# KelestZ/Latent2im

Measured on AMD Instinct MI355X. Metric: edited images/sec, higher is better.
Workload: dtype f32; 1 GPU; StyleGAN2 FFHQ-shaped 1024^2 generator (random-init, noise weights ~ 0.05: per-layer noise drawn every pass), ResNet-50 regressor, 1 CelebA attr (train.py flow), full loss (reg+content+GAN), batch 8 per GPU, linear W+ walk, eager launches; resolution=1024, global_batch=8, per_gpu_batch=8, losses=reg+content+gan, parallelism=dp1, loss_branch_streams=3, hip_graph=False

## Files before the change

include/l2i.h:

```cpp
#ifndef L2I_H
#define L2I_H

#include <stdint.h>

#ifdef __cplusplus
extern "C" {
#endif

#define L2I_OK 0
#define L2I_E_ARG (-1)
#define L2I_E_LAUNCH (-2)
#define L2I_E_UNSUPPORTED (-3)

#define L2I_ACT_NONE 0
#define L2I_ACT_LRELU 1
#define L2I_ACT_RELU 2

typedef struct l2i_conv_params {
    const float* x;
    const float* w;
    float* y;
    int32_t B, Cin, H, W, Cout, CoutP;
    int32_t KH, KW, stride, pad_y, pad_x;
    int32_t OH, OW, OHf, OWf;
// ... 28 lines not shown
    const float* rgb_bias;
    float* rgb_out;
    float* pool_out;
    uint8_t* pool_idx;
    uint8_t* mask_out;
    int32_t mask_bits;
} l2i_conv_params;
#define L2I_SQ_SLOTS 1024

int l2i_conv2d_f32(const l2i_conv_params* p, void* stream);

#define L2I_FAMILY_IMPLICIT_GEMM 0
#define L2I_FAMILY_GEMM1X1 1
#define L2I_FAMILY_CIN3 2
#define L2I_FAMILY_DIRECT_SMALL 3
int l2i_conv2d_family(const l2i_conv_params* p);

int l2i_conv_transpose2d_f32(const l2i_conv_params* p, void* stream);
#define L2I_CONVT_HINT_DIRECT 9
#define L2I_CONVT_HINT_POLY 10
#define L2I_TFAMILY_DIRECT 0
#define L2I_TFAMILY_POLY 1
#define L2I_TFAMILY_SMALL 2
int l2i_conv_transpose2d_family(const l2i_conv_params* p);
typedef struct l2i_convt_poly_plan {
    int32_t eligible, masked;
    int32_t nwx, nwy;
    int32_t WTW, WTH, tiles_x, tiles_y, mblocks;
    int32_t total, grid;
    int32_t IH, IW, org, nslots, plane, wpitch;
    int32_t CK, stage_floats, lds_bytes;
// ... 236 lines not shown
```

latent2im_amd/_lib.py:

```python
import ctypes
import os

import torch

_HERE = os.path.dirname(os.path.abspath(__file__))
LIB_PATH = os.environ.get('L2I_LIB') or os.path.join(_HERE, 'libl2i_hip.so')

ACT_NONE, ACT_LRELU, ACT_RELU = 0, 1, 2
LINEAR_NONE, LINEAR_LRELU, LINEAR_WALK = 0, 1, 2

c_f = ctypes.c_float
c_i = ctypes.c_int32
c_p = ctypes.c_void_p
c_l = ctypes.c_int64
c_d = ctypes.c_double


class ConvParams(ctypes.Structure):
    _fields_ = [
        ('x', c_p), ('w', c_p), ('y', c_p),
        ('B', c_i), ('Cin', c_i), ('H', c_i), ('W', c_i), ('Cout', c_i), ('CoutP', c_i),
        ('KH', c_i), ('KW', c_i), ('stride', c_i), ('pad_y', c_i), ('pad_x', c_i),
        ('OH', c_i), ('OW', c_i), ('OHf', c_i), ('OWf', c_i),
        ('oy_step', c_i), ('ox_step', c_i), ('oy_off', c_i), ('ox_off', c_i),
# ... 22 lines not shown

class SegmvSeg(ctypes.Structure):
    _fields_ = [('rows', c_i), ('nparts', c_i), ('out_off_c', c_i), ('out_off_b', c_i), ('out_bstride', c_i), ('epi', c_i), ('bias_off', c_i),
                ('e_off_c', c_i), ('e_off_b', c_i), ('e_bstride', c_i), ('rgb_off_b', c_i), ('rgb_w_off', c_i), ('part', SegmvPart * 2)]


CONVT_HINT_DIRECT, CONVT_HINT_POLY = 9, 10
TFAMILY_DIRECT, TFAMILY_POLY, TFAMILY_SMALL = 0, 1, 2


class ConvtPolyPlan(ctypes.Structure):
    _fields_ = [(n, c_i) for n in ('eligible', 'masked', 'nwx', 'nwy', 'WTW', 'WTH', 'tiles_x', 'tiles_y', 'mblocks', 'total', 'grid',
                                   'IH', 'IW', 'org', 'nslots', 'plane', 'wpitch', 'CK', 'stage_floats', 'lds_bytes')]


H8_EPI_LEAN, H8_EPI_GENERAL, H8_EPI_F32_VEC, H8_EPI_F32_SCALAR = 0, 1, 2, 3


class ConvH8Plan(ctypes.Structure):
    _fields_ = [(n, c_i) for n in ('eligible', 'WM', 'WN', 'KS', 'K', 'S', 'TR', 'out32', 'relu_in', 'extra', 'rgb', 'epilogue', 'nchunks', 'tiles_x',
                                   'tiles_y', 'mblocks', 'total', 'grid', 'lds_bytes')]


def conv_h8_plan(p, transposed=False):
    plan = ConvH8Plan()
    check(load().l2i_conv_h8_plan_for(ctypes.byref(p), int(bool(transposed)), ctypes.byref(plan)), 'l2i_conv_h8_plan_for')
    return plan


ADAM_MAX_TENSORS = 16
# ... 14 lines not shown

def repack_taps(taps):
    t = RepackTaps()
    t.count = len(taps)
    for i, (ky, kx) in enumerate(taps[:REPACK_MAX_TAPS]):
        t.ky[i], t.kx[i] = ky, kx
    return t


_SIGNATURES = {
    'l2i_conv2d_f32': (c_i, [ctypes.POINTER(ConvParams), c_p]),
    'l2i_conv2d_family': (c_i, [ctypes.POINTER(ConvParams)]),
    'l2i_conv_transpose2d_f32': (c_i, [ctypes.POINTER(ConvParams), c_p]),
    'l2i_conv_transpose2d_family': (c_i, [ctypes.POINTER(ConvParams)]),
    'l2i_convt_poly_plan_for': (c_i, [ctypes.POINTER(ConvParams), ctypes.POINTER(ConvtPolyPlan)]),
    'l2i_conv2d_bf16x3_f32': (c_i, [ctypes.POINTER(ConvParams), c_p]),
    'l2i_conv_transpose2d_bf16x3_f32': (c_i, [ctypes.POINTER(ConvParams), c_p]),
    'l2i_conv2d_wino_f32': (c_i, [ctypes.POINTER(ConvParams), c_p]),
    'l2i_conv2d_wino4_f32': (c_i, [ctypes.POINTER(ConvParams), c_p]),
    'l2i_wino4s_epilogue_class': (c_i, [ctypes.POINTER(ConvParams)]),
    'l2i_conv1x1_pair_f32': (c_i, [ctypes.POINTER(ConvParams), ctypes.POINTER(ConvParams), c_p]),
    'l2i_conv2d_h8': (c_i, [ctypes.POINTER(ConvParams), c_p]),
    'l2i_conv_transpose2d_h8': (c_i, [ctypes.POINTER(ConvParams), c_p]),
    'l2i_conv_h8_plan_for': (c_i, [ctypes.POINTER(ConvParams), c_i, ctypes.POINTER(ConvH8Plan)]),
    'l2i_conv_img_h8': (c_i, [ctypes.POINTER(ConvParams), c_p]),
    'l2i_conv1x1_pair_h8': (c_i, [ctypes.POINTER(ConvParams), ctypes.POINTER(ConvParams), c_i, c_p]),
    'l2i_conv_chain3_h8': (c_i, [ctypes.POINTER(ConvParams), ctypes.POINTER(ConvParams), ctypes.POINTER(ConvParams), c_i, c_p]),
    'l2i_fused_bias_act_f32': (c_i, [c_p, c_p, c_p, c_p, c_l, c_l, c_l, c_i, c_i, c_f, c_f, c_p]),
    'l2i_fused_bias_act_f16': (c_i, [c_p, c_p, c_p, c_p, c_l, c_l, c_l, c_i, c_i, c_f, c_f, c_p]),
    'l2i_upfirdn2d_f16': (c_i, [c_p, c_p, c_p, c_l, c_i, c_i, c_i, c_i, c_i, c_i, c_i, c_i, c_i, c_i, c_i, c_i, c_p]),
# ... 54 lines not shown
    'l2i_pixelnorm_act_h8': (c_i, [c_p, c_p, c_p, c_i, c_i, c_i, c_i, c_f, c_f, c_i, c_p]),
    'l2i_pixelnorm_act_bwd_h8': (c_i, [c_p, c_p, c_p, c_p, c_i, c_i, c_i, c_i, c_f, c_f, c_i, c_p]),
    'l2i_linear_rows_f32': (c_i, [c_p, c_p, c_p, c_p, c_p, c_p, c_i, c_i, c_i, c_i, c_f, c_p]),
    'l2i_linear_rows_bwd_f32': (c_i, [c_p, c_p, c_p, c_p, c_p, c_p, c_p, c_p, c_p, c_p, c_i, c_i, c_i, c_i, c_f, c_i, c_p]),
    'l2i_range_stats': (c_i, [c_p, c_p, c_l, c_i, c_p]),
    'l2i_last_error': (ctypes.c_char_p, []),
    'l2i_abi_version': (c_i, []),
    'l2i_sizeof_conv_params': (c_i, []),
}

_F16_TWINS = frozenset(k for k in _SIGNATURES if k.endswith('_h8') or k in ('l2i_cast_f32_to_h8', 'l2i_cast_h8_to_f32'))
for _n in [k for k in _SIGNATURES if k in _F16_TWINS]:
    _SIGNATURES[_n + '_f16'] = _SIGNATURES[_n]

ABI_VERSION = 12
ADDITIVE = frozenset(('l2i_conv_transpose2d_family', 'l2i_convt_poly_plan_for', 'l2i_conv_h8_plan_for', 'l2i_bn_finalize_f32', 'l2i_bn_bwd_finalize_f32',
                      'l2i_repack_taps_f32', 'l2i_repack_wino_f32', 'l2i_batch_from_u8_f32'))

EXPORTS = tuple(_SIGNATURES)

_lib = None


BUILD_HASHES = os.path.join(_HERE, 'csrc', 'BUILD_HASHES.json')


def committed_build():
    import hashlib
    import json
    try:
        with open(BUILD_HASHES) as f:
# ... 87 lines not shown
```

latent2im_amd/conv.py:

```python

import numpy as np
import torch

from . import _lib
from ._lib import ACT_LRELU, ACT_NONE, ACT_RELU, ConvParams


import os as _os

PRECISION = _os.environ.get('L2I_PRECISION', 'f32')
H8_PRECISIONS = ('bf16', 'f16')


def h8_dtype():
    return torch.float16 if PRECISION == 'f16' else torch.bfloat16

USE_WINOGRAD = True
WINO4_MODES = ('all', 'tall', 'r4', 'off')
WINO4 = 'all'
WINO4_R4_MIN_W = 64
SPLIT_K = True
_WS = {}
USE_FUSED_TRANSPOSED = True
PROFILE = None
FAMILIES = ('implicit_gemm_f32', 'gemm1x1_f32', 'cin3_f32', 'direct_small_valu')
FAMILY_INFO = {
    'winograd_f32': ('conv_wino_kernel', 16.0 / 36.0, 157.3),
    'winograd4_f32': ('conv_wino4s_kernel', 36.0 / 144.0, 157.3),
    'implicit_gemm_f32': ('conv_mfma_kernel / conv3x3s2_dma_kernel', 1.0, 157.3),
    'gemm1x1_f32': ('gemm1x1_kernel', 1.0, 157.3),
    'transposed_f32': ('convt_mfma_kernel', 1.0, 157.3),
    'transposed_poly_f32': ('convt_poly_kernel', 25.0 / 36.0, 157.3),
    'cin3_f32': ('conv_cin3_kernel', 28.0 / 27.0, 157.3),
    'direct_small_valu': ('conv_direct_small_kernel', 1.0, 157.3),
    'implicit_gemm_bf16x3': ('conv_bf16x3_pipe_kernel', 3.0, 2500.0),
    'transposed_bf16x3': ('conv_bf16x3_pipe_kernel<TR>', 3.0, 2500.0),
    'conv_h8': ('conv_h8_kernel', 1.0, 2500.0),
    'transposed_h8': ('conv_h8_kernel<TR>', 1.0, 2500.0),
}


def pack_weight(w):
    w = torch.as_tensor(w, dtype=torch.float32)
    cout, cin, kh, kw = w.shape
# ... 55 lines not shown
_POLY_G = np.array([[0, 0, 1], [1, 0, 1], [1, 0, 0], [0, 1, 0], [0, 1, 0]], dtype=np.float64)


def pack_weight_convt_poly(w, dtype=torch.float32):
    w = torch.as_tensor(w, dtype=torch.float64)
    cout, cin, kh, kw = w.shape
    assert kh == 3 and kw == 3
    G = torch.as_tensor(_POLY_G, device=w.device)
    U = torch.einsum('ik,ockl,jl->ocij', G, w, G)
    coutp = (cout + 31) // 32 * 32
    p = torch.zeros(cin, 25, coutp, dtype=dtype, device=w.device)
    p[:, :, :cout] = U.permute(1, 2, 3, 0).reshape(cin, 25, cout).to(dtype)
    return p.contiguous()


def _bf16x3_planes(self):
    if self.w16 is None and self.w_src is not None:
        hi, lo = pack_weight_bf16x3(self.w_src)
        self.w16 = (hi.to(self.w.device), lo.to(self.w.device))
    return self.w16


class Launch:
    __slots__ = ('w', 'cin', 'cout', 'kh', 'kw', 'stride', 'pad_y', 'pad_x', 'step', 'off_y', 'off_x', 'w16', 'w_src', 'wino', 'w4', 'wino4')

    def __init__(self, w_oihw, stride, pad_y, pad_x, step=1, off_y=0, off_x=0, device=None):
        self.cout, self.cin, self.kh, self.kw = w_oihw.shape
        self.w = pack_weight(w_oihw).to(device) if device is not None else pack_weight(w_oihw)
        self.stride, self.pad_y, self.pad_x = stride, pad_y, pad_x
        self.step, self.off_y, self.off_x = step, off_y, off_x
        self.w16 = None
        self.w4 = None
        if self.cout <= 4 and stride == 1:
            self.w4 = torch.zeros(self.cin, self.kh * self.kw, 4, dtype=torch.float32, device=self.w.device)
            self.w4[:, :, :self.cout] = self.w[:, :, :self.cout]
        self.wino = None
        self.wino4 = None
        self.w_src = torch.as_tensor(w_oihw, dtype=torch.float32) if (self.cin % 8 == 0 and self.kh <= 3 and self.kw <= 3) else None

    bf16x3_planes = _bf16x3_planes

    def wino_pack(self):
        if self.wino is None and self.w_src is not None and self.kh == 3 and self.kw == 3:
            self.wino = pack_weight_wino(self.w_src).to(self.w.device)
        return self.wino

    def wino4_pack(self):
        if self.wino4 is None and self.w_src is not None and self.kh == 3 and self.kw == 3:
            self.wino4 = pack_weight_wino4(self.w_src).to(self.w.device)
        return self.wino4

    def to(self, device):
        self.w = self.w.to(device)
        if self.w4 is not None:
            self.w4 = self.w4.to(device)
        if self.wino is not None:
            self.wino = self.wino.to(device)
        if self.wino4 is not None:
            self.wino4 = self.wino4.to(device)
        if self.w16 is not None:
            self.w16 = tuple(t.to(device) for t in self.w16)
        return self


def correlation_plan(w_oihw, stride, pad):
    return [Launch(torch.as_tensor(w_oihw, dtype=torch.float32), stride, pad, pad)]


def _phase_axis(K, pad, pi):
    k0 = (pi + pad) % 2
    ks = list(range(k0, K, 2))
    if not ks:
        return None, 0
    A = len(ks)
    d = (pi + pad - k0) // 2
    taps = [k0 + 2 * (A - 1 - a) for a in range(A)]
# ... 265 lines not shown
                and cin * H * W * 4 < 0x7FFF0000):
            pk = L.wino4_pack()
            p.w, p.CoutP = _lib.fptr(pk), pk.shape[1] * 16
            p.tile_hint = 1 if WINO4 == 'r4' else (2 if WINO4 == 'tall' else 0)
            if (pool is not None and WINO4 != 'r4' and L.step == 1 and OHf % 2 == 0 and OWf % 4 == 0 and OH == OHf and OW == OWf and not accumulate
                    and pool[0].data_ptr() % 8 == 0):
                assert tuple(pool[0].shape) == (B, L.cout, OHf // 2, OWf // 2) and pool[1].shape == pool[0].shape and pool[1].dtype == torch.uint8
                p.pool_out, p.pool_idx = _lib.fptr(pool[0]), _lib.ptr(pool[1])
                pool[2][0] = True
            name, family = 'l2i_conv2d_wino4_f32', 'winograd4_f32'
        else:
            p.w = _lib.fptr(L.wino_pack())
            name, family = 'l2i_conv2d_wino_f32', 'winograd_f32'
        fuse_sq = True
    elif L.kh * L.kw > 1 and L.cout > 4:
        _split_k(p, B * OH * OW, cin, y)
    if (sq is not None and sq[0].data_ptr() % 16 == 0
            and (fuse_sq or (family is None and tile_hint == 0 and p.ksplit <= 1
                             and _lib.load().l2i_conv2d_family(p) == 2))):
        _fuse_sq(p, y, sq)
    _launch(name, (p,), None, _conv_meta, p, family)


def _bf16x3_eligible(L, x, in_mask, OW):
    k1 = L.kh == 1 and L.kw == 1 and L.pad_y == 0 and L.pad_x == 0
    k3 = L.kh == 3 and L.kw == 3 and L.pad_y == L.pad_x and (L.pad_x == 1 or (L.pad_x == 0 and L.stride == 2))
    if k1 and L.stride == 1 and (in_mask is not None or L.cin * L.cout < 65536):
        return False
    return ((k1 or k3) and L.step == 1 and L.w_src is not None and L.cin % (32 if k1 else 16) == 0 and L.cout > 4 and OW >= 32
            and x.shape[3] % 4 == 0 and x.data_ptr() % 16 == 0 and (in_mask is None or in_mask.data_ptr() % 16 == 0))

# ... 22 lines not shown
        table = _TAP_TABLES[key] = _lib.repack_taps(key)
    rows, cols = (cout, cin) if swap else (cin, cout)
    colsp = dst.shape[-1] if layout == _lib.REPACK_PACKED else cols
    assert dst.numel() == rows * len(key) * colsp and dst.device == weight.device, (tuple(dst.shape), rows, len(key), colsp)
    _lib.call('l2i_repack_taps_f32', _lib.fptr(dst), _lib.fptr(weight), cout, cin, k, table, int(swap), colsp, layout)


def _repack_launch(L, weight, taps, swap, flip=None):
    _repack_taps(L.w, weight, taps, swap)
    if L.w4 is not None:
        _repack_taps(L.w4, weight, taps, swap)
    if L.w_src is not None and L.w_src.data_ptr() != weight.data_ptr():
        _repack_taps(L.w_src, weight, taps, not swap, _lib.REPACK_OIHW)
    if L.w16 is not None:
        raise _lib.L2IError('repack_: no kernel rewrites bf16x3 planes (L2I_PRECISION=bf16x3 is for frozen weights)')
    for pack, kind in ((L.wino, _lib.REPACK_WINO2), (L.wino4, _lib.REPACK_WINO4)):
        if pack is not None:
            if flip is None:
                raise _lib.L2IError('repack_: a Winograd pack on a launch that is not a whole 3x3 weight')
            cout, cin = weight.shape[:2]
            _lib.call('l2i_repack_wino_f32', _lib.fptr(pack), _lib.fptr(weight), cout, cin, kind, int(swap), int(flip))


def _weight_f32(weight, keep_cuda=False):
    w = torch.as_tensor(weight if torch.is_tensor(weight) else np.asarray(weight), dtype=torch.float32)
    return w if keep_cuda and w.is_cuda else w.cpu()


class FrozenConv2d:

# ... 291 lines not shown
```

latent2im_amd/csrc/l2i_conv.hip:

```cpp

#include <hip/hip_runtime.h>
#include <stdint.h>
#include <type_traits>
#include "l2i.h"
#include "l2i_internal.h"
#include "l2i_device.h"
#include "l2i_epilogue.h"


struct ConvLaunch {
    int tw_log2, th_log2, tb_log2;
    int tiles_x, tiles_y, bgroups, mblocks;
    int CK;
    int IH, IW, IWp;
    int planeS, plane;
    int rows_c;
    unsigned magic_iw, magic_rc, magic_ih;
    int in_elems;
    int w_vec;
    int vec_epi;
    int lstride, gstep;
    int total;
    int ksplit, cin_per;
};
// ... 671 lines not shown
    L.in_elems = ck * in_per_c;
    L.w_vec = ck * KK * BM / 4;
    L.magic_iw = magic_for((unsigned)L.IW);
    L.magic_rc = magic_for((unsigned)L.rows_c);
    L.magic_ih = magic_for((unsigned)L.IH);
    lds = per_c * ck + (size_t)(ck << L.tb_log2) * sizeof(float);
    L.vec_epi = (l2i_epilogue_vec_ok(p) && L.tw_log2 >= 2) ? 1 : 0;
    if (L.vec_epi && lds < 4 * 32 * 64 * sizeof(float)) lds = 4 * 32 * 64 * sizeof(float);
    grid = (long)L.bgroups * L.tiles_y * L.tiles_x * L.mblocks * L.ksplit;
    if (!(lds <= 64 * 1024 && grid > 0 && grid <= 0x7ffffff0L)) return false;
    L.total = (int)grid;
    grid = (grid + 7) & ~7L;
    return true;
}

extern "C" int l2i_conv2d_family(const l2i_conv_params* pp) {
    if (!pp) return L2I_E_ARG;
    const l2i_conv_params& p = *pp;
    if (p.Cout <= 4 && p.stride == 1 && p.KH <= 16 && p.tile_hint == 0 && !p.out_scale && !p.noise && !p.bias && !p.residual && !p.out_mask &&
        p.act == L2I_ACT_NONE)
        return L2I_FAMILY_DIRECT_SMALL;
    if (p.tile_hint == 0 && l2i_gemm1x1_eligible(p)) return L2I_FAMILY_GEMM1X1;
    if (p.tile_hint == 0 && l2i_cin3_eligible(p)) return L2I_FAMILY_CIN3;
    return L2I_FAMILY_IMPLICIT_GEMM;
}

extern "C" int l2i_conv2d_f32(const l2i_conv_params* pp, void* stream) {
    if (!pp) return l2i_set_error(L2I_E_ARG, "conv2d: null params");
    const l2i_conv_params& p = *pp;
    if (!p.x || !p.w || !p.y) return l2i_set_error(L2I_E_ARG, "conv2d: null tensor");
    if (const char* m = l2i_unsupported_v5_fields(p, false, false, false)) return l2i_set_error(L2I_E_UNSUPPORTED, m);
    if (p.B <= 0 || p.Cin <= 0 || p.Cout <= 0 || p.H <= 0 || p.W <= 0 || p.OH <= 0 || p.OW <= 0)
        return l2i_set_error(L2I_E_ARG, "conv2d: non-positive dimension");
    if (p.KH <= 0 || p.KW <= 0 || p.KH > 16 || p.KW > 16 || (p.stride != 1 && p.stride != 2))
        return l2i_set_error(L2I_E_ARG, "conv2d: kernel size must be 1..16 and stride 1 or 2");
    const bool dense4 = p.CoutP == 4 && p.Cout <= 4;
    if (!dense4 && (p.CoutP < p.Cout || (p.CoutP % 32) != 0)) return l2i_set_error(L2I_E_ARG, "conv2d: CoutP must be Cout rounded up to 32 (or 4 for the direct kernel of <= 4 channels)");
    if (dense4 && l2i_conv2d_family(pp) != L2I_FAMILY_DIRECT_SMALL) return l2i_set_error(L2I_E_ARG, "conv2d: the [Cin][K*K][4] pack is for launches of the direct <= 4-channel kernel only");
    if (p.res_sub && !p.residual) return l2i_set_error(L2I_E_ARG, "conv2d: res_sub needs residual");
    if ((p.sq_ref || p.sq_out) && !(p.sq_ref && p.sq_out && (((uintptr_t)p.sq_ref) % 16) == 0 && p.tile_hint == 0 && l2i_cin3_eligible(p)))
        return l2i_set_error(L2I_E_UNSUPPORTED, "conv2d: sq_ref / sq_out are fused in l2i_conv2d_wino_f32 and in the <= 3-input-channel kernel only");
    if (p.oy_step <= 0 || p.ox_step <= 0 || (p.OH - 1) * p.oy_step + p.oy_off >= p.OHf || (p.OW - 1) * p.ox_step + p.ox_off >= p.OWf ||
        p.oy_off < 0 || p.ox_off < 0)
        return l2i_set_error(L2I_E_ARG, "conv2d: output window exceeds the output tensor");
    if ((((uintptr_t)p.w) % 16) != 0) return l2i_set_error(L2I_E_ARG, "conv2d: packed weights must be 16-byte aligned");
    if ((size_t)p.Cin * p.H * p.W * sizeof(float) >= 0xFFFFFFF0ull || (size_t)p.Cin * p.KH * p.KW * p.CoutP * sizeof(float) >= 0xFFFFFFF0ull)
        return l2i_set_error(L2I_E_UNSUPPORTED, "conv2d: one sample / the weight pack must stay below 4 GiB (32-bit buffer offsets)");

    const int family = l2i_conv2d_family(pp);
    if (family == L2I_FAMILY_DIRECT_SMALL) return launch_direct_small(p, (hipStream_t)stream);
    if (family == L2I_FAMILY_GEMM1X1) return l2i_launch_gemm1x1(p, (hipStream_t)stream);
    if (family == L2I_FAMILY_CIN3) return l2i_launch_cin3(p, (hipStream_t)stream);
    if (p.tile_hint == 0 && l2i_conv3x3s2_eligible(p)) return l2i_launch_conv3x3s2(p, (hipStream_t)stream);

    ConvLaunch L, Lbest;
    bool vec = false, vbest = false;
    size_t lds = 0, lbest = 0;
    long grid = 0, gbest = -1;
    int sel = -1;
    if (p.tile_hint > 0) {
        if (p.tile_hint > kNumTiles) return l2i_set_error(L2I_E_ARG, "conv2d: tile_hint out of range");
        sel = p.tile_hint - 1;
        if (!plan_tile(p, kTiles[sel].wm, kTiles[sel].wn, Lbest, vbest, lbest, gbest))
            return l2i_set_error(L2I_E_UNSUPPORTED, "conv2d: requested tile cannot be staged for this problem");
// ... 42 lines not shown
```

latent2im_amd/csrc/l2i_convt_poly.hip:

```cpp

#include <hip/hip_runtime.h>
#include <stdint.h>
#include <string.h>
#include "l2i.h"
#include "l2i_internal.h"
#include "l2i_device.h"

namespace {

constexpr int POLY_BM = 16;
constexpr int POLY_NW = 64;
constexpr int POLY_WP = 16 * POLY_BM + 16;
constexpr int POLY_NSL = 6;
constexpr int POLY_LDS_MAX = 52 * 1024;

struct PolyLaunch {
    int WTW, WTH;
    unsigned magic_tw, magic_iw;
    int tiles_x, tiles_y, mblocks, total;
    int IH, IW, nslots, plane, CK, stage_f;
};

template <int PAD, bool MASK>
__global__ __launch_bounds__(256, 3) void convt_poly_kernel(const l2i_conv_params p, const PolyLaunch L) {
// ... 170 lines not shown
                } else {
                    d[0] = Y[0];
                    if (ox0 + 1 < p.OWf) d[1] = Y[1];
                    if (ox0 + 2 < p.OWf) d[2] = Y[2];
                }
            }
        }
    }
}

unsigned magic_of(unsigned d) { return d == 1 ? 0u : (unsigned)((0x100000000ULL + d - 1) / d); }

struct PolyRule { int pad, masked, cin, cout, h; };
constexpr PolyRule kPolyRules[] = {
    {0, 0, 512, 512, 32}, {0, 0, 512, 256, 64}, {0, 0, 256, 128, 128}, {0, 0, 128, 64, 256}, {0, 0, 64, 32, 512},
};

}

extern "C" int l2i_convt_poly_plan_for(const l2i_conv_params* pp, l2i_convt_poly_plan* plan) {
    if (!pp || !plan) return l2i_set_error(L2I_E_ARG, "convt_poly_plan: null argument");
    const l2i_conv_params& p = *pp;
    memset(plan, 0, sizeof(*plan));
    const char* why = nullptr;
    if (p.KH != 3 || p.KW != 3 || p.pad_y != p.pad_x || (p.pad_y != 0 && p.pad_y != 1)) why = "convt_poly: 3x3, pad 0 or 1 only";
    else if (p.B <= 0 || p.Cin <= 0 || p.Cout <= 0 || p.H <= 0 || p.W <= 0) why = "convt_poly: non-positive dimension";
    else if (p.in_h8) why = "convt_poly: fp32 maps only";
    else if (p.ksplit > 1 && p.ws) why = "convt_poly: no split-K";
    else if (p.W < 32) why = "convt_poly: maps at least 32 positions wide";
    else if ((p.Cin % 4) != 0) why = "convt_poly: Cin must be a multiple of 4";
// ... 82 lines not shown
```

latent2im_amd/csrc/l2i_internal.h:

```cpp
#ifndef L2I_INTERNAL_H
#define L2I_INTERNAL_H
#include <hip/hip_runtime.h>
#include <atomic>
#include <cstdint>

int l2i_set_error(int code, const char* msg);

struct l2i_conv_params;
bool l2i_gemm1x1_eligible(const l2i_conv_params& p);
int l2i_launch_gemm1x1(const l2i_conv_params& p, hipStream_t st);
bool l2i_cin3_eligible(const l2i_conv_params& p);
int l2i_launch_cin3(const l2i_conv_params& p, hipStream_t st);
bool l2i_convt_small_eligible(const l2i_conv_params& p);
int l2i_launch_convt_small(const l2i_conv_params& p, hipStream_t st);
bool l2i_conv3x3s2_eligible(const l2i_conv_params& p);
int l2i_launch_conv3x3s2(const l2i_conv_params& p, hipStream_t st);
bool l2i_convt_poly_eligible(const l2i_conv_params& p);
bool l2i_convt_poly_preferred(const l2i_conv_params& p);
int l2i_launch_convt_poly(const l2i_conv_params& p, hipStream_t st);
int l2i_launch_splitk_epilogue(const l2i_conv_params& q, hipStream_t st);

static inline const char* l2i_unsupported_v5_fields(const l2i_conv_params& p, bool allow_rgb, bool allow_pool, bool allow_in_h8) {
    if (!allow_rgb && (p.rgb_w || p.rgb_bias || p.rgb_out)) return "rgb_w / rgb_bias / rgb_out are fused in l2i_conv2d_h8 only";
    if (!allow_pool && (p.pool_out || p.pool_idx)) return "pool_out / pool_idx are fused in l2i_conv2d_wino4_f32 only";
    if (!allow_in_h8 && p.in_h8) return "in_h8 is read by the 7x7 kernel of l2i_conv_transpose2d_f32 only";
    if (!allow_rgb && (p.mask_out || p.mask_bits)) return "mask_out / mask_bits (one-bit activation masks) belong to l2i_conv2d_h8 / l2i_conv_transpose2d_h8";
    return nullptr;
}

#define L2I_CHECK_LAUNCH()                                                      \
    do {                                                                        \
        hipError_t e_ = hipGetLastError();                                      \
        if (e_ != hipSuccess) return l2i_set_error(L2I_E_LAUNCH, hipGetErrorString(e_)); \
    } while (0)
// ... 21 lines not shown
```

Before: 83.33 images/s.

## Add polyphase 25-product kernel for 3x3 stride-2 convolutions and extend convt poly rules

```diff
diff --git a/include/l2i.h b/include/l2i.h
--- a/include/l2i.h
+++ b/include/l2i.h
@@ -66,7 +66,20 @@
 #define L2I_FAMILY_GEMM1X1 1
 #define L2I_FAMILY_CIN3 2
 #define L2I_FAMILY_DIRECT_SMALL 3
+#define L2I_FAMILY_IMPLICIT_GEMM_POLY 4
 int l2i_conv2d_family(const l2i_conv_params* p);
+
+#define L2I_CONV_HINT_AUTO_DIRECT 9
+#define L2I_CONV_HINT_S2_POLY 10
+typedef struct l2i_conv_s2_poly_plan {
+    int32_t eligible, preferred, scaled;
+    int32_t nwx, nwy;
+    int32_t WTW, WTH, tiles_x, tiles_y, mblocks;
+    int32_t total, grid;
+    int32_t IH, IW, org, nslots, plane, wpitch;
+    int32_t CK, stage_floats, lds_bytes;
+} l2i_conv_s2_poly_plan;
+int l2i_conv_s2_poly_plan_for(const l2i_conv_params* p, l2i_conv_s2_poly_plan* plan);
 
 int l2i_conv_transpose2d_f32(const l2i_conv_params* p, void* stream);
 #define L2I_CONVT_HINT_DIRECT 9
diff --git a/latent2im_amd/_lib.py b/latent2im_amd/_lib.py
--- a/latent2im_amd/_lib.py
+++ b/latent2im_amd/_lib.py
@@ -60,6 +60,21 @@
                                    'IH', 'IW', 'org', 'nslots', 'plane', 'wpitch', 'CK', 'stage_floats', 'lds_bytes')]
 
 
+CONV_HINT_AUTO_DIRECT, CONV_HINT_S2_POLY = 9, 10
+FAMILY_IMPLICIT_GEMM_POLY = 4
+
+
+class ConvS2PolyPlan(ctypes.Structure):
+    _fields_ = [(n, c_i) for n in ('eligible', 'preferred', 'scaled', 'nwx', 'nwy', 'WTW', 'WTH', 'tiles_x', 'tiles_y', 'mblocks', 'total', 'grid',
+                                   'IH', 'IW', 'org', 'nslots', 'plane', 'wpitch', 'CK', 'stage_floats', 'lds_bytes')]
+
+
+def conv_s2_poly_plan(p):
+    plan = ConvS2PolyPlan()
+    check(load().l2i_conv_s2_poly_plan_for(ctypes.byref(p), ctypes.byref(plan)), 'l2i_conv_s2_poly_plan_for')
+    return plan
+
+
 H8_EPI_LEAN, H8_EPI_GENERAL, H8_EPI_F32_VEC, H8_EPI_F32_SCALAR = 0, 1, 2, 3
 
 
@@ -104,6 +119,7 @@
     'l2i_conv_transpose2d_f32': (c_i, [ctypes.POINTER(ConvParams), c_p]),
     'l2i_conv_transpose2d_family': (c_i, [ctypes.POINTER(ConvParams)]),
     'l2i_convt_poly_plan_for': (c_i, [ctypes.POINTER(ConvParams), ctypes.POINTER(ConvtPolyPlan)]),
+    'l2i_conv_s2_poly_plan_for': (c_i, [ctypes.POINTER(ConvParams), ctypes.POINTER(ConvS2PolyPlan)]),
     'l2i_conv2d_bf16x3_f32': (c_i, [ctypes.POINTER(ConvParams), c_p]),
     'l2i_conv_transpose2d_bf16x3_f32': (c_i, [ctypes.POINTER(ConvParams), c_p]),
     'l2i_conv2d_wino_f32': (c_i, [ctypes.POINTER(ConvParams), c_p]),
@@ -188,7 +204,7 @@
     _SIGNATURES[_n + '_f16'] = _SIGNATURES[_n]
 
 ABI_VERSION = 12
-ADDITIVE = frozenset(('l2i_conv_transpose2d_family', 'l2i_convt_poly_plan_for', 'l2i_conv_h8_plan_for', 'l2i_bn_finalize_f32', 'l2i_bn_bwd_finalize_f32',
+ADDITIVE = frozenset(('l2i_conv_transpose2d_family', 'l2i_convt_poly_plan_for', 'l2i_conv_s2_poly_plan_for', 'l2i_conv_h8_plan_for', 'l2i_bn_finalize_f32', 'l2i_bn_bwd_finalize_f32',
                       'l2i_repack_taps_f32', 'l2i_repack_wino_f32', 'l2i_batch_from_u8_f32'))
 
 EXPORTS = tuple(_SIGNATURES)
diff --git a/latent2im_amd/conv.py b/latent2im_amd/conv.py
--- a/latent2im_amd/conv.py
+++ b/latent2im_amd/conv.py
@@ -23,11 +23,12 @@
 _WS = {}
 USE_FUSED_TRANSPOSED = True
 PROFILE = None
-FAMILIES = ('implicit_gemm_f32', 'gemm1x1_f32', 'cin3_f32', 'direct_small_valu')
+FAMILIES = ('implicit_gemm_f32', 'gemm1x1_f32', 'cin3_f32', 'direct_small_valu', 'implicit_gemm_poly_f32')
 FAMILY_INFO = {
     'winograd_f32': ('conv_wino_kernel', 16.0 / 36.0, 157.3),
     'winograd4_f32': ('conv_wino4s_kernel', 36.0 / 144.0, 157.3),
     'implicit_gemm_f32': ('conv_mfma_kernel / conv3x3s2_dma_kernel', 1.0, 157.3),
+    'implicit_gemm_poly_f32': ('conv3x3s2_poly_kernel', 25.0 / 36.0, 157.3),
     'gemm1x1_f32': ('gemm1x1_kernel', 1.0, 157.3),
     'transposed_f32': ('convt_mfma_kernel', 1.0, 157.3),
     'transposed_poly_f32': ('convt_poly_kernel', 25.0 / 36.0, 157.3),
@@ -113,6 +114,26 @@
     return p.contiguous()
 
 
+_S2_POLY_G = np.array([[1, 0, 0], [1, 0, 1], [0, 0, 1], [0, 1, 0]], dtype=np.float64)
+
+
+def pack_weight_s2_poly(w, dtype=torch.float32):
+    w = torch.as_tensor(w, dtype=torch.float64)
+    cout, cin, kh, kw = w.shape
+    assert kh == 3 and kw == 3
+    G = torch.as_tensor(_S2_POLY_G, device=w.device)
+    U = torch.einsum('ik,ockl,jl->ocij', G, w, G)
+    coutp = (cout + 31) // 32 * 32
+    p = torch.zeros(cin, 16, coutp, dtype=dtype, device=w.device)
+    p[:, :, :cout] = U.permute(1, 2, 3, 0).reshape(cin, 16, cout).to(dtype)
+    return p.contiguous()
+
+
+def s2_poly_source(w_oihw, stride):
+    cout, cin, kh, kw = w_oihw.shape
+    return w_oihw if (kh == 3 and kw == 3 and stride == 2 and cin % 4 == 0 and w_oihw.device.type == 'cpu') else None
+
+
 def _bf16x3_planes(self):
     if self.w16 is None and self.w_src is not None:
         hi, lo = pack_weight_bf16x3(self.w_src)
@@ -121,7 +142,7 @@
 
 
 class Launch:
-    __slots__ = ('w', 'cin', 'cout', 'kh', 'kw', 'stride', 'pad_y', 'pad_x', 'step', 'off_y', 'off_x', 'w16', 'w_src', 'wino', 'w4', 'wino4')
+    __slots__ = ('w', 'cin', 'cout', 'kh', 'kw', 'stride', 'pad_y', 'pad_x', 'step', 'off_y', 'off_x', 'w16', 'w_src', 'wino', 'w4', 'wino4', 's2p_src', 's2p')
 
     def __init__(self, w_oihw, stride, pad_y, pad_x, step=1, off_y=0, off_x=0, device=None):
         self.cout, self.cin, self.kh, self.kw = w_oihw.shape
@@ -136,8 +157,15 @@
         self.wino = None
         self.wino4 = None
         self.w_src = torch.as_tensor(w_oihw, dtype=torch.float32) if (self.cin % 8 == 0 and self.kh <= 3 and self.kw <= 3) else None
+        self.s2p_src = s2_poly_source(w_oihw, stride) if (step == 1 and pad_y == pad_x and pad_y in (0, 1)) else None
+        self.s2p = None
 
     bf16x3_planes = _bf16x3_planes
+
+    def s2_poly_pack(self):
+        if self.s2p is None and self.s2p_src is not None:
+            self.s2p = pack_weight_s2_poly(self.s2p_src).to(self.w.device)
+        return self.s2p
 
     def wino_pack(self):
         if self.wino is None and self.w_src is not None and self.kh == 3 and self.kw == 3:
@@ -159,6 +187,8 @@
             self.wino4 = self.wino4.to(device)
         if self.w16 is not None:
             self.w16 = tuple(t.to(device) for t in self.w16)
+        if self.s2p is not None:
+            self.s2p = self.s2p.to(device)
         return self
 
 
@@ -454,7 +484,12 @@
             name, family = 'l2i_conv2d_wino_f32', 'winograd_f32'
         fuse_sq = True
     elif L.kh * L.kw > 1 and L.cout > 4:
-        _split_k(p, B * OH * OW, cin, y)
+        if tile_hint != _lib.CONV_HINT_S2_POLY:
+            _split_k(p, B * OH * OW, cin, y)
+        if (L.s2p_src is not None and p.ksplit <= 1 and tile_hint in (0, _lib.CONV_HINT_S2_POLY) and _lib.has('l2i_conv_s2_poly_plan_for')):
+            plan = _lib.conv_s2_poly_plan(p)
+            if plan.eligible and (plan.preferred or tile_hint):
+                p.w_lo = _lib.fptr(L.s2_poly_pack())
     if (sq is not None and sq[0].data_ptr() % 16 == 0
             and (fuse_sq or (family is None and tile_hint == 0 and p.ksplit <= 1
                              and _lib.load().l2i_conv2d_family(p) == 2))):
@@ -507,6 +542,9 @@
         _repack_taps(L.w_src, weight, taps, not swap, _lib.REPACK_OIHW)
     if L.w16 is not None:
         raise _lib.L2IError('repack_: no kernel rewrites bf16x3 planes (L2I_PRECISION=bf16x3 is for frozen weights)')
+    if L.s2p is not None:
+        raise _lib.L2IError('repack_: this convolution was packed from a host weight (16-plane pack of the 25-product stride-2 kernel); build it from a CUDA weight')
+    L.s2p_src = None
     for pack, kind in ((L.wino, _lib.REPACK_WINO2), (L.wino4, _lib.REPACK_WINO4)):
         if pack is not None:
             if flip is None:
diff --git a/latent2im_amd/csrc/l2i_conv.hip b/latent2im_amd/csrc/l2i_conv.hip
--- a/latent2im_amd/csrc/l2i_conv.hip
+++ b/latent2im_amd/csrc/l2i_conv.hip
@@ -709,9 +709,7 @@
     return true;
 }
 
-extern "C" int l2i_conv2d_family(const l2i_conv_params* pp) {
-    if (!pp) return L2I_E_ARG;
-    const l2i_conv_params& p = *pp;
+static int family_direct(const l2i_conv_params& p) {
     if (p.Cout <= 4 && p.stride == 1 && p.KH <= 16 && p.tile_hint == 0 && !p.out_scale && !p.noise && !p.bias && !p.residual && !p.out_mask &&
         p.act == L2I_ACT_NONE)
         return L2I_FAMILY_DIRECT_SMALL;
@@ -720,9 +718,24 @@
     return L2I_FAMILY_IMPLICIT_GEMM;
 }
 
+static bool takes_s2_poly(const l2i_conv_params& p) {
+    if (p.tile_hint == L2I_CONV_HINT_S2_POLY) return l2i_conv_s2_poly_eligible(p);
+    return p.tile_hint == 0 && p.w_lo && p.KH == 3 && p.KW == 3 && p.stride == 2 && family_direct(p) == L2I_FAMILY_IMPLICIT_GEMM && l2i_conv_s2_poly_preferred(p);
+}
+
+extern "C" int l2i_conv2d_family(const l2i_conv_params* pp) {
+    if (!pp) return L2I_E_ARG;
+    l2i_conv_params p = *pp;
+    if (p.tile_hint == L2I_CONV_HINT_AUTO_DIRECT) { p.tile_hint = 0; return family_direct(p); }
+    return takes_s2_poly(p) ? L2I_FAMILY_IMPLICIT_GEMM_POLY : family_direct(p);
+}
+
 extern "C" int l2i_conv2d_f32(const l2i_conv_params* pp, void* stream) {
     if (!pp) return l2i_set_error(L2I_E_ARG, "conv2d: null params");
-    const l2i_conv_params& p = *pp;
+    l2i_conv_params q = *pp;
+    const bool auto_direct = q.tile_hint == L2I_CONV_HINT_AUTO_DIRECT;
+    if (auto_direct) q.tile_hint = 0;
+    const l2i_conv_params& p = q;
     if (!p.x || !p.w || !p.y) return l2i_set_error(L2I_E_ARG, "conv2d: null tensor");
     if (const char* m = l2i_unsupported_v5_fields(p, false, false, false)) return l2i_set_error(L2I_E_UNSUPPORTED, m);
     if (p.B <= 0 || p.Cin <= 0 || p.Cout <= 0 || p.H <= 0 || p.W <= 0 || p.OH <= 0 || p.OW <= 0)
@@ -731,7 +744,7 @@
         return l2i_set_error(L2I_E_ARG, "conv2d: kernel size must be 1..16 and stride 1 or 2");
     const bool dense4 = p.CoutP == 4 && p.Cout <= 4;
     if (!dense4 && (p.CoutP < p.Cout || (p.CoutP % 32) != 0)) return l2i_set_error(L2I_E_ARG, "conv2d: CoutP must be Cout rounded up to 32 (or 4 for the direct kernel of <= 4 channels)");
-    if (dense4 && l2i_conv2d_family(pp) != L2I_FAMILY_DIRECT_SMALL) return l2i_set_error(L2I_E_ARG, "conv2d: the [Cin][K*K][4] pack is for launches of the direct <= 4-channel kernel only");
+    if (dense4 && family_direct(p) != L2I_FAMILY_DIRECT_SMALL) return l2i_set_error(L2I_E_ARG, "conv2d: the [Cin][K*K][4] pack is for launches of the direct <= 4-channel kernel only");
     if (p.res_sub && !p.residual) return l2i_set_error(L2I_E_ARG, "conv2d: res_sub needs residual");
     if ((p.sq_ref || p.sq_out) && !(p.sq_ref && p.sq_out && (((uintptr_t)p.sq_ref) % 16) == 0 && p.tile_hint == 0 && l2i_cin3_eligible(p)))
         return l2i_set_error(L2I_E_UNSUPPORTED, "conv2d: sq_ref / sq_out are fused in l2i_conv2d_wino_f32 and in the <= 3-input-channel kernel only");
@@ -742,7 +755,9 @@
     if ((size_t)p.Cin * p.H * p.W * sizeof(float) >= 0xFFFFFFF0ull || (size_t)p.Cin * p.KH * p.KW * p.CoutP * sizeof(float) >= 0xFFFFFFF0ull)
         return l2i_set_error(L2I_E_UNSUPPORTED, "conv2d: one sample / the weight pack must stay below 4 GiB (32-bit buffer offsets)");
 
-    const int family = l2i_conv2d_family(pp);
+    if (!auto_direct && takes_s2_poly(p)) return l2i_launch_conv_s2_poly(p, (hipStream_t)stream);
+    if (p.tile_hint == L2I_CONV_HINT_S2_POLY) return L2I_E_UNSUPPORTED;
+    const int family = family_direct(p);
     if (family == L2I_FAMILY_DIRECT_SMALL) return launch_direct_small(p, (hipStream_t)stream);
     if (family == L2I_FAMILY_GEMM1X1) return l2i_launch_gemm1x1(p, (hipStream_t)stream);
     if (family == L2I_FAMILY_CIN3) return l2i_launch_cin3(p, (hipStream_t)stream);
diff --git a/latent2im_amd/csrc/l2i_conv_s2_poly.hip b/latent2im_amd/csrc/l2i_conv_s2_poly.hip
--- /dev/null
+++ b/latent2im_amd/csrc/l2i_conv_s2_poly.hip
@@ -0,0 +1,255 @@
+#include <hip/hip_runtime.h>
+#include <stdint.h>
+#include <string.h>
+#include "l2i.h"
+#include "l2i_internal.h"
+#include "l2i_device.h"
+#include "l2i_epilogue.h"
+
+namespace {
+
+constexpr int SP_BM = 16;
+constexpr int SP_WTW = 16, SP_WTH = 4;
+constexpr int SP_IH = 4 * SP_WTH + 1;
+constexpr int SP_IW = 4 * SP_WTW + 1;
+constexpr int SP_XCOL = SP_IH * 64;
+constexpr int SP_NSL = SP_IH + 1;
+constexpr int SP_PLANE = SP_NSL * 64 + 16;
+constexpr int SP_WP = 16 * SP_BM + 16;
+constexpr int SP_CK = 4;
+constexpr int SP_W_OFF = SP_CK * SP_PLANE, SP_SC_OFF = SP_W_OFF + SP_CK * SP_WP;
+constexpr int SP_STAGE = SP_SC_OFF + 64;
+constexpr int SP_LDS_BYTES = 2 * SP_STAGE * (int)sizeof(float);
+constexpr int SP_LDS_MAX = 52 * 1024;
+static_assert(SP_PLANE % 32 == 16 && SP_WP % 32 == 16 && SP_LDS_BYTES <= SP_LDS_MAX && SP_XCOL + SP_IH <= SP_NSL * 64, "bank offsets / three blocks per CU");
+
+struct S2PolyLaunch {
+    int tiles_x, tiles_y, mblocks, total;
+};
+
+template <bool SCALE>
+__global__ __launch_bounds__(256, 3) void conv3x3s2_poly_kernel(const l2i_conv_params p, const S2PolyLaunch L) {
+    extern __shared__ __attribute__((aligned(16))) float smem[];
+    const int tid = threadIdx.x, lane = tid & 63, kq = lane >> 4, nl = lane & 15;
+    const int wave = __builtin_amdgcn_readfirstlane(tid >> 6);
+    int bid = (int)((blockIdx.x & 7) * (gridDim.x >> 3) + (blockIdx.x >> 3));
+    if (bid >= L.total) return;
+    const int mblk = __builtin_amdgcn_readfirstlane(bid % L.mblocks); bid /= L.mblocks;
+    const int tx = __builtin_amdgcn_readfirstlane(bid % L.tiles_x); bid /= L.tiles_x;
+    const int ty = __builtin_amdgcn_readfirstlane(bid % L.tiles_y);
+    const int b = __builtin_amdgcn_readfirstlane(bid / L.tiles_y);
+    const int m0 = mblk * SP_BM;
+    const int wy0 = ty * SP_WTH, wx0 = tx * SP_WTW;
+    const int iy0 = 4 * wy0 - p.pad_y, ix0 = 4 * wx0 - p.pad_x;
+
+    f32x4 acc[25];
+#pragma unroll
+    for (int q = 0; q < 25; ++q) acc[q] = f32x4{0.f, 0.f, 0.f, 0.f};
+
+    const size_t plane_x = (size_t)p.H * p.W;
+    const unsigned in_bytes = (unsigned)((size_t)p.Cin * plane_x * sizeof(float));
+    const __amdgpu_buffer_rsrc_t rs_x = l2i_buffer_rsrc(p.x + (size_t)b * p.Cin * plane_x, in_bytes);
+    const unsigned wrow_b = (unsigned)p.CoutP * 16u * (unsigned)sizeof(float);
+    const __amdgpu_buffer_rsrc_t rs_w = l2i_buffer_rsrc(p.w_lo, (unsigned)p.Cin * wrow_b);
+    const __amdgpu_buffer_rsrc_t rs_s = l2i_buffer_rsrc((SCALE ? p.in_scale : p.x) + (size_t)b * p.Cin, SCALE ? (unsigned)(p.Cin * sizeof(float)) : 0u);
+    constexpr unsigned OOB = 0x80000000u;
+
+    const int gxr = ix0 + 4 * nl + kq;
+    const unsigned vrow = (gxr >= 0 && gxr < p.W) ? (unsigned)gxr * 4u : OOB;
+    const int gyc = iy0 + lane, gxc = ix0 + 64;
+    const unsigned vcol = (lane < SP_IH && gyc >= 0 && gyc < p.H && gxc < p.W) ? (unsigned)(gyc * p.W + gxc) * 4u : OOB;
+    const unsigned wvoff = (unsigned)(((lane >> 2) * p.CoutP + m0 + (lane & 3) * 4) * sizeof(float));
+    const unsigned scoff = (lane < SP_CK) ? (unsigned)(lane * sizeof(float)) : OOB;
+
+    auto dma = [&](int c0, int st) {
+        const unsigned lds0 = l2i_lds_addr(smem + st * SP_STAGE);
+        const unsigned c = (unsigned)(c0 + wave);
+        l2i_lds_dma16(wvoff, rs_w, __builtin_amdgcn_readfirstlane(lds0 + (unsigned)((SP_W_OFF + wave * SP_WP) * 4)), c * wrow_b);
+        const unsigned base = __builtin_amdgcn_readfirstlane(lds0 + (unsigned)(wave * SP_PLANE * 4));
+        const unsigned so = c * (unsigned)(plane_x * sizeof(float));
+#pragma unroll
+        for (int s = 0; s < SP_IH; ++s) {
+            const int gy = iy0 + s;
+            const bool ok = gy >= 0 && gy < p.H;
+            l2i_lds_dma4(ok ? vrow : OOB, rs_x, base + (unsigned)(s * 256), ok ? so + (unsigned)(gy * p.W) * 4u : so);
+        }
+        l2i_lds_dma4(vcol, rs_x, base + (unsigned)(SP_XCOL * 4), so);
+        if constexpr (SCALE) {
+            if (wave == 0) l2i_lds_dma4(scoff, rs_s, __builtin_amdgcn_readfirstlane(lds0 + (unsigned)(SP_SC_OFF * 4)), (unsigned)(c0 * sizeof(float)));
+        }
+    };
+
+    const int wlane = SP_W_OFF + kq * SP_WP + nl;
+    const int rlane = kq * SP_PLANE + 4 * wave * 64 + nl;
+    const int r4lane = kq * SP_PLANE + (nl < 15 ? 4 * wave * 64 + nl + 1 : SP_XCOL + 4 * wave);
+    const int r4step = nl < 15 ? 64 : 1;
+
+    auto mfma_chunk = [&](int st) {
+        const float* sp = smem + st * SP_STAGE;
+        float sv = 1.f;
+        if constexpr (SCALE) sv = sp[SP_SC_OFF + kq];
+        auto column = [&](int j, float (&v)[5]) {
+            float r[5];
+#pragma unroll
+            for (int i = 0; i < 5; ++i) {
+                r[i] = j < 4 ? sp[rlane + i * 64 + j * 16] : sp[r4lane + i * r4step];
+                if constexpr (SCALE) r[i] *= sv;
+            }
+            v[0] = r[0] - r[2]; v[1] = r[2]; v[2] = r[2] - r[4]; v[3] = r[1]; v[4] = r[3];
+        };
+        auto planes = [&](int bcol, float (&a)[4]) {
+#pragma unroll
+            for (int q = 0; q < 4; ++q) a[q] = sp[wlane + (q * 4 + bcol) * SP_BM];
+        };
+        auto products = [&](int c, const float (&a)[4], const float (&t)[5]) {
+            constexpr int aidx[5] = {0, 1, 2, 3, 3};
+#pragma unroll
+            for (int r = 0; r < 5; ++r) acc[r * 5 + c] = __builtin_amdgcn_mfma_f32_16x16x4f32(a[aidx[r]], t[r], acc[r * 5 + c], 0, 0, 0);
+        };
+        float a[4], v[5], v2[5], t[5];
+        planes(3, a);
+        column(1, v); products(3, a, v);
+        column(3, v); products(4, a, v);
+        planes(1, a);
+        column(2, v2); products(1, a, v2);
+        planes(0, a);
+        column(0, v);
+#pragma unroll
+        for (int r = 0; r < 5; ++r) t[r] = v[r] - v2[r];
+        products(0, a, t);
+        planes(2, a);
+        column(4, v);
+#pragma unroll
+        for (int r = 0; r < 5; ++r) t[r] = v2[r] - v[r];
+        products(2, a, t);
+    };
+
+    dma(0, 0);
+    __builtin_amdgcn_s_waitcnt(0x0F70);
+    __syncthreads();
+    int st = 0;
+    for (int c0 = 0; c0 < p.Cin; c0 += SP_CK, st ^= 1) {
+        const bool next = c0 + SP_CK < p.Cin;
+        if (next) dma(c0 + SP_CK, st ^ 1);
+        mfma_chunk(st);
+        __builtin_amdgcn_s_waitcnt(0x0F70);
+        __syncthreads();
+    }
+
+    const int oy0 = 2 * (wy0 + wave), ox0 = 2 * (wx0 + nl);
+    if (oy0 >= p.OH || ox0 >= p.OW) return;
+    const bool two = ox0 + 1 < p.OW;
+    const size_t plane_o = (size_t)p.OHf * p.OWf;
+    const float* osc = p.out_scale ? p.out_scale + (size_t)b * p.Cout : nullptr;
+#pragma unroll
+    for (int r = 0; r < 4; ++r) {
+        const int co = m0 + kq * 4 + r;
+        if (co >= p.Cout) continue;
+        float R[2][5];
+#pragma unroll
+        for (int c = 0; c < 5; ++c) {
+            R[0][c] = (acc[0 * 5 + c][r] + acc[1 * 5 + c][r]) + acc[3 * 5 + c][r];
+            R[1][c] = (acc[1 * 5 + c][r] - acc[2 * 5 + c][r]) + acc[4 * 5 + c][r];
+        }
+        const size_t obase = ((size_t)b * p.Cout + co) * plane_o + (size_t)oy0 * p.OWf + ox0;
+#pragma unroll
+        for (int i = 0; i < 2; ++i) {
+            if (oy0 + i >= p.OH) continue;
+            const size_t oidx = obase + (size_t)i * p.OWf;
+            float y0 = (R[i][0] + R[i][1]) + R[i][3], y1 = (R[i][1] - R[i][2]) + R[i][4];
+            if (osc) { y0 *= osc[co]; y1 *= osc[co]; }
+            if (p.out_mask) {
+                if (two) {
+                    const float2 mk = *reinterpret_cast<const float2*>(p.out_mask + oidx);
+                    y0 = epi_keep(y0, mk.x); y1 = epi_keep(y1, mk.y);
+                } else {
+                    y0 = epi_keep(y0, p.out_mask[oidx]);
+                }
+            }
+            if (p.bias) { y0 += p.bias[co]; y1 += p.bias[co]; }
+            y0 = epi_act_select(p, y0); y1 = epi_act_select(p, y1);
+            if (p.out_gain != 1.f) { y0 *= p.out_gain; y1 *= p.out_gain; }
+            if (two) *reinterpret_cast<float2*>(p.y + oidx) = make_float2(y0, y1);
+            else p.y[oidx] = y0;
+        }
+    }
+}
+
+struct S2PolyRule { int pad, scaled, cin, cout, h; };
+constexpr S2PolyRule kS2PolyRules[] = {
+    {-1, 0, 0, 0, 0},
+};
+
+}
+
+extern "C" int l2i_conv_s2_poly_plan_for(const l2i_conv_params* pp, l2i_conv_s2_poly_plan* plan) {
+    if (!pp || !plan) return l2i_set_error(L2I_E_ARG, "conv_s2_poly_plan: null argument");
+    const l2i_conv_params& p = *pp;
+    memset(plan, 0, sizeof(*plan));
+    const char* why = nullptr;
+    if (p.KH != 3 || p.KW != 3 || p.stride != 2 || p.pad_y != p.pad_x || (p.pad_y != 0 && p.pad_y != 1)) why = "conv_s2_poly: 3x3 stride 2, pad 0 or 1 only";
+    else if (p.B <= 0 || p.Cin <= 0 || p.Cout <= 0 || p.H <= 0 || p.W <= 0 || p.OH <= 0 || p.OW <= 0) why = "conv_s2_poly: non-positive dimension";
+    else if (p.in_mask) why = "conv_s2_poly: in_mask is not fused";
+    else if (p.sq_ref || p.sq_out) why = "conv_s2_poly: sq_ref is not fused";
+    else if (p.ws || p.ksplit > 1) why = "conv_s2_poly: no split-K";
+    else if (p.noise || p.residual || p.res_mask || p.res_sub || p.accumulate) why = "conv_s2_poly: noise / residual / res_mask / res_sub / accumulate are not fused";
+    else if (p.oy_step != 1 || p.ox_step != 1 || p.oy_off != 0 || p.ox_off != 0) why = "conv_s2_poly: dense output window at the origin only";
+    else if (p.OH > p.OHf || p.OW > p.OWf) why = "conv_s2_poly: output window exceeds the output tensor";
+    else if (l2i_unsupported_v5_fields(p, false, false, false)) why = "conv_s2_poly: fp32 maps and the fp32 epilogue only";
+    else if ((p.Cin % 4) != 0) why = "conv_s2_poly: Cin must be a multiple of 4";
+    else if (p.CoutP < p.Cout || (p.CoutP % 32) != 0) why = "conv_s2_poly: CoutP must be Cout rounded up to 32";
+    else if ((size_t)p.Cin * p.H * p.W * sizeof(float) >= 0x7FFF0000ull) why = "conv_s2_poly: sample >= 2 GiB";
+    else if ((size_t)p.Cin * 16 * p.CoutP * sizeof(float) >= 0xFFFFFFF0ull) why = "conv_s2_poly: weight pack >= 4 GiB";
+    if (why) { l2i_set_error(L2I_E_UNSUPPORTED, why); return L2I_OK; }
+    plan->scaled = p.in_scale ? 1 : 0;
+    plan->nwx = (p.OW + 1) / 2;
+    plan->nwy = (p.OH + 1) / 2;
+    plan->WTW = SP_WTW; plan->WTH = SP_WTH;
+    plan->tiles_x = (plan->nwx + SP_WTW - 1) / SP_WTW;
+    plan->tiles_y = (plan->nwy + SP_WTH - 1) / SP_WTH;
+    plan->mblocks = (p.Cout + SP_BM - 1) / SP_BM;
+    plan->IH = SP_IH; plan->IW = SP_IW;
+    plan->org = -p.pad_y;
+    plan->nslots = SP_NSL;
+    plan->plane = SP_PLANE;
+    plan->wpitch = SP_WP;
+    plan->CK = SP_CK;
+    plan->stage_floats = SP_STAGE;
+    plan->lds_bytes = SP_LDS_BYTES;
+    const long total = (long)p.B * plan->tiles_y * plan->tiles_x * plan->mblocks;
+    if (total <= 0 || total > 0x7ffffff0L) { l2i_set_error(L2I_E_UNSUPPORTED, "conv_s2_poly: grid too large"); return L2I_OK; }
+    plan->total = (int)total;
+    plan->grid = (int)((total + 7) & ~7L);
+    plan->eligible = 1;
+    if (p.H == p.W)
+        for (const S2PolyRule& r : kS2PolyRules)
+            if (r.pad == p.pad_y && r.scaled == plan->scaled && r.cin == p.Cin && r.cout == p.Cout && r.h == p.H) plan->preferred = 1;
+    return L2I_OK;
+}
+
+bool l2i_conv_s2_poly_eligible(const l2i_conv_params& p) {
+    l2i_conv_s2_poly_plan plan;
+    return l2i_conv_s2_poly_plan_for(&p, &plan) == L2I_OK && plan.eligible;
+}
+
+bool l2i_conv_s2_poly_preferred(const l2i_conv_params& p) {
+    l2i_conv_s2_poly_plan plan;
+    return l2i_conv_s2_poly_plan_for(&p, &plan) == L2I_OK && plan.eligible && plan.preferred;
+}
+
+template <bool SCALE>
+static int launch_s2_poly(const l2i_conv_params& p, const l2i_conv_s2_poly_plan& plan, hipStream_t st) {
+    S2PolyLaunch L;
+    L.tiles_x = plan.tiles_x; L.tiles_y = plan.tiles_y; L.mblocks = plan.mblocks; L.total = plan.total;
+    L2I_ONCE_PER_DEVICE((void)hipFuncSetAttribute(reinterpret_cast<const void*>(&conv3x3s2_poly_kernel<SCALE>), hipFuncAttributeMaxDynamicSharedMemorySize, SP_LDS_MAX));
+    hipLaunchKernelGGL((conv3x3s2_poly_kernel<SCALE>), dim3((unsigned)plan.grid), dim3(256), (size_t)plan.lds_bytes, st, p, L);
+    L2I_CHECK_LAUNCH();
+    return L2I_OK;
+}
+
+int l2i_launch_conv_s2_poly(const l2i_conv_params& p, hipStream_t st) {
+    l2i_conv_s2_poly_plan plan;
+    if (l2i_conv_s2_poly_plan_for(&p, &plan) != L2I_OK || !plan.eligible) return L2I_E_UNSUPPORTED;
+    if (!p.w_lo || (((uintptr_t)p.w_lo) % 16) != 0) return l2i_set_error(L2I_E_ARG, "conv_s2_poly: w_lo must be the 16-byte aligned [Cin][16][CoutP] pack");
+    return p.in_scale ? launch_s2_poly<true>(p, plan, st) : launch_s2_poly<false>(p, plan, st);
+}
diff --git a/latent2im_amd/csrc/l2i_convt_poly.hip b/latent2im_amd/csrc/l2i_convt_poly.hip
--- a/latent2im_amd/csrc/l2i_convt_poly.hip
+++ b/latent2im_amd/csrc/l2i_convt_poly.hip
@@ -208,6 +208,7 @@
 struct PolyRule { int pad, masked, cin, cout, h; };
 constexpr PolyRule kPolyRules[] = {
     {0, 0, 512, 512, 32}, {0, 0, 512, 256, 64}, {0, 0, 256, 128, 128}, {0, 0, 128, 64, 256}, {0, 0, 64, 32, 512},
+    {1, 1, 128, 128, 128}, {1, 1, 256, 256, 64}, {1, 1, 512, 512, 32},
 };
 
 }
diff --git a/latent2im_amd/csrc/l2i_internal.h b/latent2im_amd/csrc/l2i_internal.h
--- a/latent2im_amd/csrc/l2i_internal.h
+++ b/latent2im_amd/csrc/l2i_internal.h
@@ -18,6 +18,9 @@
 bool l2i_convt_poly_eligible(const l2i_conv_params& p);
 bool l2i_convt_poly_preferred(const l2i_conv_params& p);
 int l2i_launch_convt_poly(const l2i_conv_params& p, hipStream_t st);
+bool l2i_conv_s2_poly_eligible(const l2i_conv_params& p);
+bool l2i_conv_s2_poly_preferred(const l2i_conv_params& p);
+int l2i_launch_conv_s2_poly(const l2i_conv_params& p, hipStream_t st);
 int l2i_launch_splitk_epilogue(const l2i_conv_params& q, hipStream_t st);
 
 static inline const char* l2i_unsupported_v5_fields(const l2i_conv_params& p, bool allow_rgb, bool allow_pool, bool allow_in_h8) {
```

Result: slower. 82.27 images/s (-1.3%).
